# smdesai/mlx-swift-audio

Measured on AMD Instinct MI355X. Metric: audio-sec/s (Whisper large-v3-turbo b=32) at 1/2/4/8 GPU; codec samples/s, higher is better.
Workload: dtype bf16; 1 GPU; Whisper large-v3-turbo bf16, batch=32x30 s synthetic clips per MI355X, log-mel+encode+greedy decode (T=0, timestamps, max_tokens 448, one window per clip), random-init N(0,0.02^2) weights; clips_per_gpu=32, global_batch=32, parallelism=dp1, replicas=3, exchange=none, schedule=pipelined

## Files before the change

mlx-swift-audio_amd/csrc/decode_kernels.hip:

```cpp
#include <cstdlib>

#include <type_traits>
#include "decode.h"

constexpr int ROW_NV = 2;

__device__ __forceinline__ float block256_sum(float v, float* sh) {
  v = wave_sum(v);
  __syncthreads();
  if ((threadIdx.x & 63) == 0) sh[threadIdx.x >> 6] = v;
  __syncthreads();
  return (sh[0] + sh[1]) + (sh[2] + sh[3]);
}

template <typename T>
__device__ __forceinline__ void row_layernorm_store(const f32x4 (&v)[ROW_NV], int nv, int D, const float* __restrict__ gamma,
                                                    const float* __restrict__ beta, uint16_t* __restrict__ h, int row, float* sh) {
  const int tid = threadIdx.x;
  f32x4 gm[ROW_NV], bt[ROW_NV];
#pragma unroll
  for (int i = 0; i < ROW_NV; ++i) {
    const bool in = tid + 256 * i < nv;
    gm[i] = in ? *reinterpret_cast<const f32x4*>(gamma + 4 * (tid + 256 * i)) : (f32x4){0.f, 0.f, 0.f, 0.f};
    bt[i] = in ? *reinterpret_cast<const f32x4*>(beta + 4 * (tid + 256 * i)) : (f32x4){0.f, 0.f, 0.f, 0.f};
// ... 495 lines not shown
  uint32_t wo[NT];
#pragma unroll
  for (int t = 0; t < NT; ++t) wo[t] = wbuf.offset(wp[t]);
  const uint32_t wsb = (uint32_t)ws * 2u;
  int am0 = m0 + r; am0 = am0 < a.M ? am0 : a.M - 1;
  int am1 = m0 + 16 + r; am1 = am1 < a.M ? am1 : a.M - 1;
  const uint16_t* ap0 = a.A + (int64_t)am0 * a.lda + kbeg + 8 * c;
  const uint16_t* ap1 = a.A + (int64_t)am1 * a.lda + kbeg + 8 * c;
  const bool av0 = m0 + r < a.M, av1 = m0 + 16 + r < a.M;
  const s16x8 zfrag = (s16x8){0, 0, 0, 0, 0, 0, 0, 0};
  s16x8 fw[NSTEP][NT], fa0[NSTEP], fa1[NSTEP];
#pragma unroll
  for (int u = 0; u < NSTEP; ++u) {
#pragma unroll
    for (int n = 0; n < NT; ++n) fw[u][n] = wbuf.template load<2>(wo[n] + (uint32_t)u * wsb);
    fa0[u] = zfrag; fa1[u] = zfrag;
    if (av0) fa0[u] = *reinterpret_cast<const s16x8*>(ap0 + 32 * u);
    if (av1) fa1[u] = *reinterpret_cast<const s16x8*>(ap1 + 32 * u);
  }
  __builtin_amdgcn_sched_barrier(0);
  skinny_rstd_prepare(a, rs, m0, wave, lane);
  f32x4 acc[NT][2];
#pragma unroll
  for (int t = 0; t < NT; ++t) { acc[t][0] = (f32x4){0.f, 0.f, 0.f, 0.f}; acc[t][1] = (f32x4){0.f, 0.f, 0.f, 0.f}; }
#pragma unroll
  for (int u = 0; u < NSTEP; ++u)
#pragma unroll
    for (int n = 0; n < NT; ++n) {
      acc[n][0] = T::mfma16(fw[u][n], fa0[u], acc[n][0]);
      acc[n][1] = T::mfma16(fw[u][n], fa1[u], acc[n][1]);
    }
  if (!skinny_wave_reduce<NT, NW>(acc, wave, lane)) return;
  skinny_store<T, MODE, NT>(a, acc, n0, m0, split, lane, rs);
}

template <typename T>
__global__ __launch_bounds__(256) void dec_lnfold(const uint16_t* __restrict__ w, int N, int K, const float* __restrict__ gamma,
                                                  const float* __restrict__ beta, float* __restrict__ c1, float* __restrict__ c2,
                                                  const float* __restrict__ bias) {
  const int lane = threadIdx.x & 63, row = blockIdx.x * 4 + (threadIdx.x >> 6);
  if (row >= N) return;
  const uint16_t* wr = w + (int64_t)row * K;
  float s1 = 0.f, s2 = 0.f;
  for (int k = lane; k < K; k += 64) { const float v = T::to_f32(wr[k]); s1 = fmaf(v, gamma[k], s1); s2 = fmaf(v, beta[k], s2); }
  s1 = wave_sum(s1); s2 = wave_sum(s2);
  if (lane == 0) { c1[row] = s1; c2[row] = s2 + (bias ? bias[row] : 0.f); }
}

int dec_launch_lnfold(const void* w16, int N, int K, const float* gamma, const float* beta, float* c1, float* c2, int dtype, hipStream_t s, const float* bias) {
  if (!w16 || !gamma || !beta || !c1 || !c2 || N <= 0 || K <= 0) return -1;
  if (dtype == MIA_F16) hipLaunchKernelGGL(dec_lnfold<F16>, dim3((N + 3) / 4), dim3(256), 0, s, (const uint16_t*)w16, N, K, gamma, beta, c1, c2, bias);
  else hipLaunchKernelGGL(dec_lnfold<BF16>, dim3((N + 3) / 4), dim3(256), 0, s, (const uint16_t*)w16, N, K, gamma, beta, c1, c2, bias);
  return hipGetLastError() == hipSuccess ? 0 : -1;
}

template <typename T>
__global__ __launch_bounds__(256) void repack_wfrag(const uint16_t* __restrict__ src, uint16_t* __restrict__ dst, int N, int K) {
  const int64_t chunk = (int64_t)blockIdx.x * 256 + threadIdx.x;
  const int ksteps = K >> 5;
  const int64_t total = (int64_t)((N + 15) >> 4) * ksteps * 64;
  if (chunk >= total) return;
  const int lane = (int)(chunk & 63);
  const int64_t tk = chunk >> 6;
  const int kstep = (int)(tk % ksteps), tile = (int)(tk / ksteps);
  const int n = tile * 16 + (lane & 15), k = kstep * 32 + 8 * (lane >> 4);
  s16x8 v = (s16x8){0, 0, 0, 0, 0, 0, 0, 0};
  if (n < N) v = *reinterpret_cast<const s16x8*>(src + (int64_t)n * K + k);
  *reinterpret_cast<s16x8*>(dst + chunk * 8) = v;
}

int dec_launch_repack_wfrag(const void* src, void* dst, int N, int K, hipStream_t s) {
  if (N <= 0 || K <= 0 || K % 32 != 0) return -1;
  const int64_t total = (int64_t)((N + 15) / 16) * (K / 32) * 64;
  hipLaunchKernelGGL(repack_wfrag<BF16>, dim3((unsigned)((total + 255) / 256)), dim3(256), 0, s, (const uint16_t*)src, (uint16_t*)dst, N, K);
  return hipGetLastError() == hipSuccess ? 0 : -1;
}

template <int NW>
struct LnStat {
  static constexpr int RPS = NW >= 8 ? 1 : 8 / NW;
  static constexpr int MAXU = 8;
  f32x2 v[MAXU][RPS];
  int j0, rows;
  bool on;
  __device__ __forceinline__ void issue(const SkinnyArgs& a, int m0, int wave, int lane) {
    on = a.ss_in != nullptr && a.c1 != nullptr;
    const int rg = lane >> 4, l16 = lane & 15;
    j0 = (wave * 4 + rg) * RPS;
    rows = a.M - m0 < 32 ? a.M - m0 : 32;
#pragma unroll
    for (int u = 0; u < MAXU; ++u)
#pragma unroll
      for (int i = 0; i < RPS; ++i) v[u][i] = (f32x2){0.f, 0.f};
    if (!on) return;
    const f32x2* ss = reinterpret_cast<const f32x2*>(a.ss_in);
#pragma unroll
    for (int u = 0; u < MAXU; ++u) {
      const int t = l16 + 16 * u;
      if (t < a.ss_tiles) {
        if (RPS >= 2 && (a.M & 1) == 0) {
#pragma unroll
          for (int i = 0; i + 1 < RPS; i += 2)
            if (j0 + i < rows) {
              const f32x4 p = *reinterpret_cast<const f32x4*>(ss + (int64_t)t * a.M + m0 + j0 + i);
              v[u][i] = (f32x2){p[0], p[1]}; v[u][i + 1] = (f32x2){p[2], p[3]};
            }
        } else {
#pragma unroll
          for (int i = 0; i < RPS; ++i)
            if (j0 + i < rows) v[u][i] = ss[(int64_t)t * a.M + m0 + j0 + i];
        }
      }
    }
  }
  __device__ __forceinline__ void finish(const SkinnyArgs& a, float* st, int lane) {
    if (!on) return;
    const int l16 = lane & 15;
#pragma unroll
    for (int i = 0; i < RPS; ++i) {
      float v1 = 0.f, v2 = 0.f;
#pragma unroll
      for (int u = 0; u < MAXU; ++u) { v1 += v[u][i][0]; v2 += v[u][i][1]; }
      v1 += dpp_f32<0xB1>(v1); v1 += dpp_f32<0x4E>(v1); v1 += dpp_f32<0x141>(v1); v1 += dpp_f32<0x140>(v1);
      v2 += dpp_f32<0xB1>(v2); v2 += dpp_f32<0x4E>(v2); v2 += dpp_f32<0x141>(v2); v2 += dpp_f32<0x140>(v2);
      const int j = j0 + i;
      if (l16 == 0 && j < rows) {
        const float mean = v1 / (float)a.ss_dim;
        const float var = fmaxf(v2 / (float)a.ss_dim - mean * mean, 0.f);
        st[2 * j] = mean; st[2 * j + 1] = rsqrtf(var + a.eps);
      }
    }
  }
};

template <typename T, int NT>
__device__ __forceinline__ void skinny_resid_frag(const SkinnyArgs& a, const f32x4 (&acc)[NT][2], int n0, int m0, int lane) {
  const int r = lane & 15, c = lane >> 4;
#pragma unroll
  for (int t = 0; t < NT; ++t) {
    const int n = n0 + 16 * t + 4 * c;
    const f32x4 gv = *reinterpret_cast<const f32x4*>(a.nw + n);
    f32x4 bv = (f32x4){0.f, 0.f, 0.f, 0.f};
    if (a.bias) bv = *reinterpret_cast<const f32x4*>(a.bias + n);
#pragma unroll
    for (int mt = 0; mt < 2; ++mt) {
      const int m = m0 + mt * 16 + r;
      float s1 = 0.f, s2 = 0.f;
      if (m < a.M) {
        float* xp = a.xres + (int64_t)m * a.N + n;
        f32x4 x = *reinterpret_cast<const f32x4*>(xp);
#pragma unroll
        for (int j = 0; j < 4; ++j) { x[j] += acc[t][mt][j] + bv[j]; s1 += x[j]; s2 += x[j] * x[j]; }
        *reinterpret_cast<f32x4*>(xp) = x;
        *reinterpret_cast<u32x2*>(reinterpret_cast<uint16_t*>(a.out) + afrag_index(m, n, a.N)) =
            (u32x2){pack2<T>(x[0] * gv[0], x[1] * gv[1]), pack2<T>(x[2] * gv[2], x[3] * gv[3])};
      }
      const float a1 = __shfl(s1, r + 16, 64), a2 = __shfl(s1, r + 32, 64), a3 = __shfl(s1, r + 48, 64);
      const float b1 = __shfl(s2, r + 16, 64), b2 = __shfl(s2, r + 32, 64), b3 = __shfl(s2, r + 48, 64);
      if (c == 0 && m < a.M)
        *reinterpret_cast<f32x2*>(a.ss_out + ((int64_t)((n0 >> 4) + t) * a.M + m) * 2) = (f32x2){((s1 + a1) + a2) + a3, ((s2 + b1) + b2) + b3};
    }
  }
}

template <typename T, int MODE, int NT, int NSTEP, int NW>
__global__ __launch_bounds__(64 * NW) void dec_skinny_fflat(SkinnyArgs a) {
  __shared__ float st[64];
  const int lane = threadIdx.x & 63, wave = threadIdx.x >> 6;
  const int split = blockIdx.y, z = blockIdx.z;
  LnStat<NW> lnstat;
  lnstat.issue(a, z * 32, wave, lane);
  const int ksteps = a.K >> 5, tiles = (a.N + 15) >> 4;
  const int ks0 = (split * NW + wave) * NSTEP;
  const uint16_t* wp[NT];
#pragma unroll
  for (int t = 0; t < NT; ++t) {
    int tile = blockIdx.x * NT + t; tile = tile < tiles ? tile : tiles - 1;
    wp[t] = a.W + (((int64_t)tile * ksteps + ks0) * 64 + lane) * 8;
  }
  const uint16_t* ap = a.A + ((((int64_t)z * ksteps + ks0) * 2) * 64 + lane) * 8;
  const SkinnyPre<NT> pre = skinny_prefetch<MODE, NT>(a, blockIdx.x * (16 * NT), z * 32, lane);
  s16x8 fw[NSTEP][NT], fa0[NSTEP], fa1[NSTEP];
  const WFragBuf wb(a);
  const WFragBuf ab(a, 0);
  const uint32_t ao = ab.offset(ap);
  uint32_t wo[NT];
#pragma unroll
  for (int t = 0; t < NT; ++t) wo[t] = wb.offset(wp[t]);
  auto load_all = [&](auto keep_tag) {
    constexpr int AUX = decltype(keep_tag)::value ? 0 : 2;
#pragma unroll
    for (int u = 0; u < NSTEP; ++u) {
#pragma unroll
      for (int n = 0; n < NT; ++n) fw[u][n] = wb.template load<AUX>(wo[n] + 1024u * u);
      fa0[u] = ab.template load<0>(ao + 2048u * u);
      fa1[u] = ab.template load<0>(ao + 2048u * u + 1024u);
    }
  };
  if (a.w_keep) load_all(std::true_type{}); else load_all(std::false_type{});
  __builtin_amdgcn_sched_barrier(0);
  lnstat.finish(a, st, lane);
  f32x4 acc[NT][2];
#pragma unroll
  for (int t = 0; t < NT; ++t) { acc[t][0] = (f32x4){0.f, 0.f, 0.f, 0.f}; acc[t][1] = (f32x4){0.f, 0.f, 0.f, 0.f}; }
#pragma unroll
  for (int u = 0; u < NSTEP; ++u)
#pragma unroll
    for (int n = 0; n < NT; ++n) {
      acc[n][0] = T::mfma16(fw[u][n], fa0[u], acc[n][0]);
      acc[n][1] = T::mfma16(fw[u][n], fa1[u], acc[n][1]);
    }
  if (!skinny_wave_reduce<NT, NW>(acc, wave, lane)) return;
  if constexpr (MODE == SK_RESID) skinny_resid_frag<T, NT>(a, acc, blockIdx.x * (16 * NT), z * 32, lane);
  else skinny_epilogue_v<T, MODE, NT>(a, acc, pre, blockIdx.x * (16 * NT), z * 32, split, lane, st);
}

template <typename T, int MODE, int NT, int KB, int NW>
__global__ __launch_bounds__(64 * NW) void dec_skinny_fring(SkinnyArgs a) {
  __shared__ float st[64];
  const int lane = threadIdx.x & 63, wave = threadIdx.x >> 6;
  const int split = blockIdx.y, z = blockIdx.z;
  LnStat<NW> lnstat;
  lnstat.issue(a, z * 32, wave, lane);
  const int ksteps = a.K >> 5, tiles = (a.N + 15) >> 4;
  const int per_wave = ksteps / (a.S * NW);
  const int ks0 = (split * NW + wave) * per_wave;
  const uint16_t* wp[NT];
#pragma unroll
  for (int t = 0; t < NT; ++t) {
    int tile = blockIdx.x * NT + t; tile = tile < tiles ? tile : tiles - 1;
    wp[t] = a.W + (((int64_t)tile * ksteps + ks0) * 64 + lane) * 8;
  }
  const uint16_t* ap = a.A + ((((int64_t)z * ksteps + ks0) * 2) * 64 + lane) * 8;
  const SkinnyPre<NT> pre = skinny_prefetch<MODE, NT>(a, blockIdx.x * (16 * NT), z * 32, lane);
  f32x4 acc[NT][2];
#pragma unroll
  for (int t = 0; t < NT; ++t) { acc[t][0] = (f32x4){0.f, 0.f, 0.f, 0.f}; acc[t][1] = (f32x4){0.f, 0.f, 0.f, 0.f}; }
  struct Batch { s16x8 w[KB][NT], a0[KB], a1[KB]; };
  const bool keep = a.w_keep != 0;
  const WFragBuf wb(a);
  const WFragBuf ab(a, 0);
  const uint32_t ao = ab.offset(ap);
  uint32_t wo[NT];
#pragma unroll
  for (int t = 0; t < NT; ++t) wo[t] = wb.offset(wp[t]);
  auto load_batch = [&](Batch& t, int ks) {
    auto go = [&](auto keep_tag) {
      constexpr int AUX = decltype(keep_tag)::value ? 0 : 2;
#pragma unroll
      for (int u = 0; u < KB; ++u) {
#pragma unroll
        for (int n = 0; n < NT; ++n) t.w[u][n] = wb.template load<AUX>(wo[n] + 1024u * (uint32_t)(ks + u));
        t.a0[u] = ab.template load<0>(ao + 2048u * (uint32_t)(ks + u));
        t.a1[u] = ab.template load<0>(ao + 2048u * (uint32_t)(ks + u) + 1024u);
      }
    };
    if (keep) go(std::true_type{}); else go(std::false_type{});
  };
  auto mma_batch = [&](const Batch& t) {
#pragma unroll
    for (int u = 0; u < KB; ++u)
#pragma unroll
      for (int n = 0; n < NT; ++n) {
        acc[n][0] = T::mfma16(t.w[u][n], t.a0[u], acc[n][0]);
        acc[n][1] = T::mfma16(t.w[u][n], t.a1[u], acc[n][1]);
      }
  };
  const int nb = per_wave / KB;
  int ks = 0;
  if (nb > 0) {
    Batch b0, b1, b2, b3;
    load_batch(b0, 0);
    if (nb > 1) load_batch(b1, KB);
    if (nb > 2) load_batch(b2, 2 * KB);
    lnstat.finish(a, st, lane);
    for (int i = 0; i < nb; i += 4) {
      if (i + 3 < nb) load_batch(b3, (i + 3) * KB);
      mma_batch(b0);
      if (i + 1 >= nb) break;
      if (i + 4 < nb) load_batch(b0, (i + 4) * KB);
      mma_batch(b1);
      if (i + 2 >= nb) break;
      if (i + 5 < nb) load_batch(b1, (i + 5) * KB);
      mma_batch(b2);
      if (i + 3 >= nb) break;
      if (i + 6 < nb) load_batch(b2, (i + 6) * KB);
      mma_batch(b3);
    }
    ks = nb * KB;
  } else lnstat.finish(a, st, lane);
  for (; ks < per_wave; ++ks) {
    const s16x8 fa0 = *reinterpret_cast<const s16x8*>(ap + 1024 * ks);
    const s16x8 fa1 = *reinterpret_cast<const s16x8*>(ap + 1024 * ks + 512);
#pragma unroll
    for (int n = 0; n < NT; ++n) {
      const s16x8 fw = *reinterpret_cast<const s16x8*>(wp[n] + 512 * ks);
      acc[n][0] = T::mfma16(fw, fa0, acc[n][0]);
      acc[n][1] = T::mfma16(fw, fa1, acc[n][1]);
    }
  }
  if (!skinny_wave_reduce<NT, NW>(acc, wave, lane)) return;
  if constexpr (MODE == SK_RESID) skinny_resid_frag<T, NT>(a, acc, blockIdx.x * (16 * NT), z * 32, lane);
  else skinny_epilogue_v<T, MODE, NT>(a, acc, pre, blockIdx.x * (16 * NT), z * 32, split, lane, st);
}

struct QFrag { const uint32_t* wfrag; const float* stfrag; };

template <typename T> struct QMagic;
template <> struct QMagic<BF16> { static constexpr uint32_t pair = 0x43004300u; static constexpr uint32_t one = 0x3f803f80u; };
template <> struct QMagic<F16> { static constexpr uint32_t pair = 0x64006400u; static constexpr uint32_t one = 0x3c003c00u; };

template <typename T, int MODE, int NT>
__device__ __forceinline__ void skinny_store_tr(const SkinnyArgs& a, const f32x4 (&acc)[NT][2], int n0, int m0, int split, int lane, const float* rs) {
  const int r = lane & 15, c = lane >> 4;
  const bool scaled = a.ss_in != nullptr;
#pragma unroll
  for (int t = 0; t < NT; ++t) {
    const int n = n0 + 16 * t + r;
    const bool nv = n < a.N;
    const float bs = (MODE != SK_PARTIAL && a.bias && nv) ? a.bias[n] : 0.f;
    const float wn = (MODE == SK_RESID && nv) ? a.nw[n] : 0.f;
#pragma unroll
    for (int mt = 0; mt < 2; ++mt) {
#pragma unroll
      for (int i = 0; i < 4; ++i) {
        const int mr = 16 * mt + 4 * c + i, m = m0 + mr;
        const bool mv = m < a.M;
        const float raw = scaled ? acc[t][mt][i] * (mv ? rs[mr] : 0.f) : acc[t][mt][i];
        float v = raw + bs;
        if (MODE == SK_SWIGLU) {
          const float u = dpp_f32<0xB1>(v);
          if (nv && mv && !(r & 1)) reinterpret_cast<uint16_t*>(a.out)[(int64_t)m * a.ldo + (n >> 1)] = T::from_f32((v / (1.0f + __expf(-v))) * u);
          continue;
        }
        if (MODE == SK_RESID) {
          float x = 0.f;
          if (nv && mv) {
            float* xp = a.xres + (int64_t)m * a.N + n;
            x = *xp + v;
            *xp = x;
            reinterpret_cast<uint16_t*>(a.out)[(int64_t)m * a.ldo + n] = T::from_f32(x * wn);
          }
          float q = x * x;
          q += dpp_f32<0xB1>(q); q += dpp_f32<0x4E>(q); q += dpp_f32<0x141>(q); q += dpp_f32<0x140>(q);
          if (r == 0 && mv) a.ss_out[(int64_t)((n0 >> 4) + t) * a.M + m] = q;
          continue;
        }
        if (!nv || !mv) continue;
        if (MODE == SK_PARTIAL) reinterpret_cast<float*>(a.out)[((int64_t)split * a.M + m) * a.N + n] = raw;
        else if (MODE == SK_OUTF32) reinterpret_cast<float*>(a.out)[(int64_t)m * a.ldo + n] = v;
        else reinterpret_cast<uint16_t*>(a.out)[(int64_t)m * a.ldo + n] = T::from_f32(v);
      }
    }
  }
}

template <typename T, int MODE, int NT, int NW, bool M16, int NP>
__global__ __launch_bounds__(64 * NW) void skinny_gemm_qi(SkinnyArgs a, QFrag q) {
  __shared__ float rs[32];
  const int lane = threadIdx.x & 63;
  const int wave = __builtin_amdgcn_readfirstlane(threadIdx.x >> 6);
  const int tile0 = blockIdx.x * NT;
  const int n0 = tile0 * 16;
  const int split = blockIdx.y;
  const int m0 = blockIdx.z * 32;
  const int nblk = a.K >> 7;
  const int bc = nblk / (a.S * NW);
  const int b0 = (split * NW + wave) * bc;
  const int n_tiles = (a.N + 15) >> 4;
  const int r = lane & 15, c = lane >> 4;
  const bool av0 = m0 + r < a.M, av1 = !M16 && m0 + 16 + r < a.M;
  const uint16_t* ap0 = a.A + (int64_t)(av0 ? m0 + r : 0) * a.lda + 8 * c;
  const uint16_t* ap1 = a.A + (int64_t)(av1 ? m0 + 16 + r : 0) * a.lda + 8 * c;
  const u32x4* wp[NT];
  const f32x4* sp[NT];
#pragma unroll
  for (int t = 0; t < NT; ++t) {
    const int tl = tile0 + t < n_tiles ? tile0 + t : n_tiles - 1;
    wp[t] = reinterpret_cast<const u32x4*>(q.wfrag) + ((int64_t)tl * nblk) * (NP * 64) + lane;
    sp[t] = reinterpret_cast<const f32x4*>(q.stfrag) + ((int64_t)tl * nblk) * 16 + r;
  }
  const __amdgpu_buffer_rsrc_t rw = __builtin_amdgcn_make_buffer_rsrc(const_cast<uint32_t*>(q.wfrag), (short)0, (int)((unsigned)n_tiles * (unsigned)nblk * (NP * 64 * 16u)), 0x00020000);
  const __amdgpu_buffer_rsrc_t rst = __builtin_amdgcn_make_buffer_rsrc(const_cast<float*>(q.stfrag), (short)0, (int)((unsigned)n_tiles * (unsigned)nblk * 256u), 0x00020000);
  uint32_t wo[NT], so[NT];
#pragma unroll
  for (int t = 0; t < NT; ++t) {
    wo[t] = (uint32_t)((const char*)wp[t] - (const char*)q.wfrag);
    so[t] = (uint32_t)((const char*)sp[t] - (const char*)q.stfrag);
  }
  f32x4 acc[NT][2];
#pragma unroll
  for (int t = 0; t < NT; ++t) { acc[t][0] = (f32x4){0.f, 0.f, 0.f, 0.f}; acc[t][1] = (f32x4){0.f, 0.f, 0.f, 0.f}; }
  const s16x8 zfrag = (s16x8){0, 0, 0, 0, 0, 0, 0, 0};
  struct Blk { u32x4 w[NT][NP]; f32x4 st[NT]; s16x8 a0[4], a1[4]; };
  auto load_blk = [&](Blk& b, int blk) {
#pragma unroll
    for (int t = 0; t < NT; ++t) {
#pragma unroll
      for (int p = 0; p < NP; ++p) b.w[t][p] = __builtin_bit_cast(u32x4, __builtin_amdgcn_raw_buffer_load_b128(rw, (int)(wo[t] + (uint32_t)(blk * NP + p) * 1024u), 0, 2));
      b.st[t] = __builtin_bit_cast(f32x4, __builtin_amdgcn_raw_buffer_load_b128(rst, (int)(so[t] + (uint32_t)blk * 256u), 0, 2));
    }
#pragma unroll
    for (int st = 0; st < 4; ++st) {
      b.a0[st] = zfrag;
      if (av0) b.a0[st] = *reinterpret_cast<const s16x8*>(ap0 + (int64_t)blk * 128 + 32 * st);
      if (!M16) { b.a1[st] = zfrag; if (av1) b.a1[st] = *reinterpret_cast<const s16x8*>(ap1 + (int64_t)blk * 128 + 32 * st); }
    }
  };
  const f32x4 zero4 = (f32x4){0.f, 0.f, 0.f, 0.f};
  const s16x8 ones = __builtin_bit_cast(s16x8, (u32x4){QMagic<T>::one, QMagic<T>::one, QMagic<T>::one, QMagic<T>::one});
  auto unpack = [](uint32_t word) -> s16x8 {
    return __builtin_bit_cast(s16x8, (u32x4){(word & 0x000f000fu) | QMagic<T>::pair, ((word >> 4) & 0x000f000fu) | QMagic<T>::pair,
                                             ((word >> 8) & 0x000f000fu) | QMagic<T>::pair, ((word >> 12) & 0x000f000fu) | QMagic<T>::pair});
  };
  auto mma_blk = [&](const Blk& b) {
#pragma unroll
    for (int g = 0; g < 2; ++g) {
      f32x4 A0 = T::mfma16(b.a0[2 * g], ones, zero4), A1 = zero4;
      A0 = T::mfma16(b.a0[2 * g + 1], ones, A0);
      if (!M16) { A1 = T::mfma16(b.a1[2 * g], ones, zero4); A1 = T::mfma16(b.a1[2 * g + 1], ones, A1); }
#pragma unroll
      for (int t = 0; t < NT; ++t) {
        f32x4 P0[NP], P1[NP];
#pragma unroll
        for (int p = 0; p < NP; ++p) {
          const s16x8 f0 = unpack(b.w[t][p][2 * g]), f1 = unpack(b.w[t][p][2 * g + 1]);
          P0[p] = T::mfma16(b.a0[2 * g], f0, zero4);
          P0[p] = T::mfma16(b.a0[2 * g + 1], f1, P0[p]);
          if (!M16) { P1[p] = T::mfma16(b.a1[2 * g], f0, zero4); P1[p] = T::mfma16(b.a1[2 * g + 1], f1, P1[p]); }
        }
        const float sc = b.st[t][2 * g], tt = b.st[t][2 * g + 1];
#pragma unroll
        for (int i = 0; i < 4; ++i) {
          const float p0 = NP == 2 ? __builtin_fmaf(16.0f, P0[NP - 1][i], P0[0][i]) : P0[0][i];
          acc[t][0][i] = __builtin_fmaf(sc, p0, __builtin_fmaf(tt, A0[i], acc[t][0][i]));
          if (!M16) {
            const float p1 = NP == 2 ? __builtin_fmaf(16.0f, P1[NP - 1][i], P1[0][i]) : P1[0][i];
            acc[t][1][i] = __builtin_fmaf(sc, p1, __builtin_fmaf(tt, A1[i], acc[t][1][i]));
          }
        }
      }
    }
  };
  Blk k0, k1, k2;
  if (bc > 0) load_blk(k0, b0);
  if (bc > 1) load_blk(k1, b0 + 1);
  skinny_rstd_prepare(a, rs, m0, wave, lane);
  for (int i = 0; i < bc; i += 3) {
    if (i + 2 < bc) load_blk(k2, b0 + i + 2);
    mma_blk(k0);
    if (i + 1 >= bc) break;
    if (i + 3 < bc) load_blk(k0, b0 + i + 3);
    mma_blk(k1);
    if (i + 2 >= bc) break;
    if (i + 4 < bc) load_blk(k1, b0 + i + 4);
    mma_blk(k2);
  }
  if (!skinny_wave_reduce<NT, NW>(acc, wave, lane)) return;
  skinny_store_tr<T, MODE, NT>(a, acc, n0, m0, split, lane, rs);
}

constexpr int DEC_MAX_KEYS = 1536;

template <typename T, int U, bool NTL>
__global__ __launch_bounds__(256) void dec_attention(const uint16_t* __restrict__ q, const uint16_t* __restrict__ kc,
                                                     const uint16_t* __restrict__ vc, uint16_t* __restrict__ out,
                                                     const int32_t* __restrict__ pos_arr, int fixed_keys, int cap_keys, int H,
                                                     float scale, float* __restrict__ qk_out, const int32_t* __restrict__ head_slot,
                                                     int n_slots, int qk_ctx) {
  __shared__ float sc[DEC_MAX_KEYS];
  __shared__ float red[4][64];
  __shared__ float red2[8];
  const int tid = threadIdx.x, lane = tid & 63, wave = tid >> 6;
  const int h = blockIdx.x, b = blockIdx.y;
  const int D = H * 64;
  const int nk = fixed_keys > 0 ? fixed_keys : pos_arr[b] + 1;
  const int c = lane & 7, g = lane >> 3;
  const uint16_t* kb = kc + ((int64_t)b * H + h) * cap_keys * 64;
  const uint16_t* vb = vc + ((int64_t)b * H + h) * cap_keys * 64;
  float qf[8];
  {
    const s16x8 qv = *reinterpret_cast<const s16x8*>(q + (int64_t)b * D + h * 64 + c * 8);
#pragma unroll
    for (int j = 0; j < 8; ++j) qf[j] = T::to_f32((uint16_t)qv[j]);
  }
  const __amdgpu_buffer_rsrc_t rk = __builtin_amdgcn_make_buffer_rsrc(const_cast<uint16_t*>(kb), (short)0, cap_keys * 128, 0x00020000);
  const __amdgpu_buffer_rsrc_t rv = __builtin_amdgcn_make_buffer_rsrc(const_cast<uint16_t*>(vb), (short)0, cap_keys * 128, 0x00020000);
  auto load_trip = [&](s16x8 (&dst)[U], const __amdgpu_buffer_rsrc_t& base, int k0) {
#pragma unroll
    for (int u = 0; u < U; ++u) {
      int key = k0 + 8 * u + g; key = key < nk ? key : nk - 1;
      dst[u] = __builtin_bit_cast(s16x8, __builtin_amdgcn_raw_buffer_load_b128(base, key * 128 + c * 16, 0, NTL ? 2 : 0));
    }
  };
  constexpr int TRIP = 32 * U;
  {
    int k0 = wave * (8 * U);
    s16x8 kv[U], kn[U];
    if (k0 < nk) load_trip(kv, rk, k0);
    for (; k0 < nk; k0 += TRIP) {
      const bool more = k0 + TRIP < nk;
      if (more) load_trip(kn, rk, k0 + TRIP);
#pragma unroll
      for (int u = 0; u < U; ++u) {
        float dot = 0.f;
#pragma unroll
        for (int j = 0; j < 8; ++j) dot += qf[j] * T::to_f32((uint16_t)kv[u][j]);
        dot += dpp_xor1(dot);
        dot += dpp_xor2(dot);
        dot += dpp_half_mirror(dot);
        const int key = k0 + 8 * u + g;
        if (c == 0 && key < nk) sc[key] = dot * scale;
      }
      if (more) {
#pragma unroll
        for (int u = 0; u < U; ++u) kv[u] = kn[u];
      }
    }
  }
  s16x8 vv[U], vn[U];
  if (wave * (8 * U) < nk) load_trip(vv, rv, wave * (8 * U));
  __syncthreads();
  if (qk_out && head_slot[h] >= 0) {
    float* dst = qk_out + (((int64_t)b * n_slots + head_slot[h]) * qk_ctx + pos_arr[b]) * nk;
    for (int i = tid; i < nk; i += 256) dst[i] = sc[i];
  }
  float m = -INFINITY;
  for (int i = tid; i < nk; i += 256) m = fmaxf(m, sc[i]);
  m = wave_max(m);
  if (lane == 0) red2[wave] = m;
  __syncthreads();
  m = fmaxf(fmaxf(red2[0], red2[1]), fmaxf(red2[2], red2[3]));
  float sum = 0.f;
  for (int i = tid; i < nk; i += 256) { const float p = __expf(sc[i] - m); sc[i] = p; sum += p; }
  sum = wave_sum(sum);
  if (lane == 0) red2[4 + wave] = sum;
  __syncthreads();
  sum = (red2[4] + red2[5]) + (red2[6] + red2[7]);
  float acc[8];
#pragma unroll
  for (int j = 0; j < 8; ++j) acc[j] = 0.f;
  for (int k0 = wave * (8 * U); k0 < nk; k0 += TRIP) {
    const bool more = k0 + TRIP < nk;
    if (more) load_trip(vn, rv, k0 + TRIP);
    float pw[U];
#pragma unroll
    for (int u = 0; u < U; ++u) {
      const int key = k0 + 8 * u + g;
      pw[u] = key < nk ? sc[key] : 0.f;
    }
#pragma unroll
    for (int u = 0; u < U; ++u)
#pragma unroll
      for (int j = 0; j < 8; ++j) acc[j] += pw[u] * T::to_f32((uint16_t)vv[u][j]);
    if (more) {
#pragma unroll
      for (int u = 0; u < U; ++u) vv[u] = vn[u];
    }
  }
#pragma unroll
  for (int j = 0; j < 8; ++j) {
    acc[j] += dpp_xor8(acc[j]);
    acc[j] += __shfl_xor(acc[j], 16, 64);
    acc[j] += __shfl_xor(acc[j], 32, 64);
  }
  if (g == 0) {
#pragma unroll
    for (int j = 0; j < 8; ++j) red[wave][c * 8 + j] = acc[j];
  }
  __syncthreads();
  if (tid < 64) {
    const float o = ((red[0][tid] + red[1][tid]) + (red[2][tid] + red[3][tid])) / sum;
    out[afrag_index(b, h * 64 + tid, D)] = T::from_f32(o);
  }
}

struct HeadBufs {
  const float* logits;
  int32_t* tokens;
  int32_t* n_gen;
  int32_t* finished;
  int32_t* last_ts;
  float* sum_logprob;
  int32_t* n_logprob;
  float* no_speech;
  const uint32_t* suppress;
  const float* uniforms;
  DecClip clip;
};

constexpr int HEAD_NPT = 52;
struct ArgMax { float v; int i; };
__device__ __forceinline__ ArgMax amax(ArgMax a, ArgMax b) {
  return (b.v > a.v || (b.v == a.v && b.i < a.i)) ? b : a;
}
__device__ __forceinline__ ArgMax wave_amax(ArgMax a) {
#define AMAX_STEP(CTRL) { const ArgMax b{dpp_f32<CTRL>(a.v), dpp_i32<CTRL>(a.i)}; a = amax(a, b); }
  AMAX_STEP(0xB1) AMAX_STEP(0x4E) AMAX_STEP(0x141) AMAX_STEP(0x140)
#undef AMAX_STEP
  ArgMax r = ArgMax{lane_f32(a.v, 0), __builtin_amdgcn_readlane(a.i, 0)};
  r = amax(r, ArgMax{lane_f32(a.v, 16), __builtin_amdgcn_readlane(a.i, 16)});
  r = amax(r, ArgMax{lane_f32(a.v, 32), __builtin_amdgcn_readlane(a.i, 32)});
  r = amax(r, ArgMax{lane_f32(a.v, 48), __builtin_amdgcn_readlane(a.i, 48)});
  return r;
}

// ... 224 lines not shown
#pragma unroll
  for (int u = 0; u < HEAD_NPT2; ++u) { const int i = base + tid + 256 * u; x[u] = i < V ? lg[i] : -INFINITY; }
  const HeadRule r = head_rule(hb, p, b);
  if (!r.active) return;
  const int nw = (V + 31) / 32;
  const uint32_t* bits = hb.suppress + (r.num_gen == 0 ? nw : 0);
  auto maskedA = [&](int i) -> bool {
    if ((bits[i >> 5] >> (i & 31)) & 1u) return true;
    if (p.timestamps) {
      if (i == p.no_timestamps) return true;
      if (r.sup_ts_all && i >= tsb) return true;
      if (r.sup_text_below_eot && i < p.eot) return true;
      if (i >= tsb && i < r.ts_floor) return true;
      if (r.sup_below_tsb && i < tsb) return true;
      if (i > r.max_first) return true;
    }
    return false;
  };
  float mx_text = -INFINITY, mx_ts = -INFINITY;
  ArgMax bA{-INFINITY, 0x7fffffff}, bB{-INFINITY, 0x7fffffff};
  unsigned okA = 0u;
#pragma unroll
  for (int u = 0; u < HEAD_NPT2; ++u) {
    const int i = base + tid + 256 * u;
    if (i >= V) continue;
    if (i >= tsb) mx_ts = fmaxf(mx_ts, x[u]); else mx_text = fmaxf(mx_text, x[u]);
    if (r.decide && !maskedA(i)) {
      okA |= 1u << u;
      bA = amax(bA, ArgMax{x[u], i});
      if (i >= tsb) bB = amax(bB, ArgMax{x[u], i});
    }
  }
  mx_text = wave_max(mx_text); mx_ts = wave_max(mx_ts);
  bA = wave_amax(bA); bB = wave_amax(bB);
  if (lane == 0) { shf[wave][0] = mx_text; shf[wave][1] = mx_ts; sha[wave][0] = bA.v; shai[wave][0] = bA.i; sha[wave][1] = bB.v; shai[wave][1] = bB.i; }
  __syncthreads();
  mx_text = shf[0][0]; mx_ts = shf[0][1]; bA = ArgMax{sha[0][0], shai[0][0]}; bB = ArgMax{sha[0][1], shai[0][1]};
  for (int w2 = 1; w2 < 4; ++w2) {
    mx_text = fmaxf(mx_text, shf[w2][0]); mx_ts = fmaxf(mx_ts, shf[w2][1]);
    bA = amax(bA, ArgMax{sha[w2][0], shai[w2][0]}); bB = amax(bB, ArgMax{sha[w2][1], shai[w2][1]});
  }
  const float mx_all = fmaxf(mx_text, mx_ts);
  __syncthreads();
  float s_all = 0.f, s_ts = 0.f, fA = 0.f, fB = 0.f;
#pragma unroll
  for (int u = 0; u < HEAD_NPT2; ++u) {
    const int i = base + tid + 256 * u;
    if (i >= V) continue;
    s_all += __expf(x[u] - mx_all);
    if (r.heuristic && i >= tsb) s_ts += __expf(x[u] - mx_ts);
    if ((okA >> u) & 1u) {
      fA += __expf(x[u] - bA.v);
      if (r.heuristic && i >= tsb) fB += __expf(x[u] - bB.v);
    }
  }
  s_all = wave_sum(s_all); s_ts = wave_sum(s_ts); fA = wave_sum(fA); fB = wave_sum(fB);
  if (lane == 0) { shf[wave][0] = s_all; shf[wave][1] = s_ts; shf[wave][2] = fA; shf[wave][3] = fB; }
  __syncthreads();
  if (tid == 0) {
    s_all = s_ts = fA = fB = 0.f;
    for (int w2 = 0; w2 < 4; ++w2) { s_all += shf[w2][0]; s_ts += shf[w2][1]; fA += shf[w2][2]; fB += shf[w2][3]; }
    parts[b * HEAD_SPLIT + k] = HeadPart{mx_text, mx_ts, s_all, s_ts, bA.v, bB.v, fA, fB, bA.i, bB.i};
  }
}

struct NextEmbed { const uint16_t* emb; const float* pos_emb; const float* gamma; const float* beta; float* x; uint16_t* h; int D; };

template <typename T>
__global__ __launch_bounds__(256) void dec_head_final(HeadBufs hb, DecodeParams p, const HeadPart* __restrict__ parts, NextEmbed ne) {
  __shared__ int s_newpos;
  __shared__ float sh[4];
  const int b = blockIdx.x, tid = threadIdx.x;
  float mx_text = -INFINITY, mx_ts = -INFINITY, s_all = 0.f, s_ts = 0.f, fA = 0.f, fB = 0.f;
  ArgMax bA{-INFINITY, 0x7fffffff}, bB{-INFINITY, 0x7fffffff};
  const HeadRule r = head_rule(hb, p, b);
  if (tid < 64 && r.active) {
    HeadPart me{-INFINITY, -INFINITY, 0.f, 0.f, -INFINITY, -INFINITY, 0.f, 0.f, 0x7fffffff, 0x7fffffff};
    if (tid < HEAD_SPLIT) me = parts[b * HEAD_SPLIT + tid];
    mx_text = wave_max(me.mx_text); mx_ts = wave_max(me.mx_ts);
    bA = wave_amax(ArgMax{me.bAv, me.bAi}); bB = wave_amax(ArgMax{me.bBv, me.bBi});
    const float mx_all = fmaxf(mx_text, mx_ts);
    const float ml = fmaxf(me.mx_text, me.mx_ts);
    s_all = wave_sum(ml > -INFINITY ? me.s_all * __expf(ml - mx_all) : 0.f);
    s_ts = wave_sum(me.mx_ts > -INFINITY ? me.s_ts * __expf(me.mx_ts - mx_ts) : 0.f);
    fA = wave_sum(me.bAv > -INFINITY ? me.fA * __expf(me.bAv - bA.v) : 0.f);
    fB = wave_sum(me.bBv > -INFINITY ? me.fB * __expf(me.bBv - bB.v) : 0.f);
  }
  if (tid == 0) {
    int newpos = -1;
    const int pos = hb.clip.pos[b];
    const int n_initial = hb.clip.n_init[b], sot_index = hb.clip.sot_idx[b];
    if (!r.active) {
      if (r.cur_len < n_initial) newpos = pos + 1;
    } else {
      const int V = p.V, tsb = p.timestamp_begin;
      const float* lg = hb.logits + (int64_t)b * V;
      int32_t* toks = hb.tokens + (int64_t)b * p.n_ctx;
      const float mx_all = fmaxf(mx_text, mx_ts);
      const float lse = mx_all + __logf(s_all);
      if (pos == sot_index) hb.no_speech[b] = __expf(lg[p.no_speech] - lse);
      if (!r.decide) newpos = pos + 1;
      else {
        bool useB = false;
        if (r.heuristic) {
          const float ts_lse = (mx_ts - lse) + __logf(s_ts);
          const float max_text = mx_text - lse;
          useB = ts_lse > max_text;
        }
        const ArgMax best = useB ? bB : bA;
        const float fsum = useB ? fB : fA;
        const bool all_masked = best.i == 0x7fffffff;
        const int next = all_masked ? 0 : best.i;
        if (next != p.eot) {
          hb.sum_logprob[b] += all_masked ? __int_as_float(0x7fc00000) : (lg[next] - best.v) - __logf(fsum);
          hb.n_logprob[b] += 1;
        }
        toks[r.cur_len] = next;
        hb.n_gen[b] = r.num_gen + 1;
        if (next > tsb) hb.last_ts[b] = next;
        int cap = p.max_tokens - n_initial;
        if (p.max_new_tokens > 0 && p.max_new_tokens < cap) cap = p.max_new_tokens;
        if (next == p.eot || r.num_gen + 1 >= cap) hb.finished[b] = 1;
        else newpos = pos + 1;
      }
    }
    if (newpos >= 0) hb.clip.pos[b] = newpos;
    s_newpos = newpos;
  }
  __syncthreads();
  const int np_ = s_newpos;
  if (np_ < 0 || np_ >= p.n_ctx) return;
  const int D = ne.D, nv = D >> 2;
  const int tok = hb.tokens[(int64_t)b * p.n_ctx + np_];
  const uint16_t* e = ne.emb + (int64_t)tok * D;
  const float* pe = ne.pos_emb + (int64_t)np_ * D;
  float* xr = ne.x + (int64_t)b * D;
  f32x4 v[ROW_NV];
#pragma unroll
  for (int i = 0; i < ROW_NV; ++i) {
    const int c = tid + 256 * i;
    if (c < nv) {
      const s16x4 ev = *reinterpret_cast<const s16x4*>(e + 4 * c);
      const f32x4 pv = *reinterpret_cast<const f32x4*>(pe + 4 * c);
#pragma unroll
      for (int j = 0; j < 4; ++j) v[i][j] = T::to_f32((uint16_t)ev[j]) + pv[j];
      *reinterpret_cast<f32x4*>(xr + 4 * c) = v[i];
    } else v[i] = (f32x4){0.f, 0.f, 0.f, 0.f};
  }
  row_layernorm_store<T>(v, nv, D, ne.gamma, ne.beta, ne.h, b, sh);
}

__global__ void dec_finalize(const int32_t* __restrict__ tokens, const int32_t* __restrict__ n_gen,
                             const float* __restrict__ sum_lp, const int32_t* __restrict__ n_lp, int32_t* __restrict__ out_tokens,
                             int32_t* __restrict__ out_n, float* __restrict__ out_avg, const int32_t* __restrict__ n_init, DecodeParams p) {
  const int b = blockIdx.x;
  const int32_t* t = tokens + (int64_t)b * p.n_ctx + n_init[b];
  __shared__ int n_keep;
  if (threadIdx.x == 0) {
    int n = n_gen[b];
    for (int i = 0; i < n; ++i) if (t[i] == p.eot) { n = i; break; }
    n_keep = n;
    out_n[b] = n;
    out_avg[b] = n_lp[b] > 0 ? sum_lp[b] / (float)n_lp[b] : 0.0f;
  }
  __syncthreads();
  for (int i = threadIdx.x; i < p.max_tokens; i += blockDim.x) out_tokens[(int64_t)b * p.max_tokens + i] = i < n_keep ? t[i] : 0;
}

int dec_launch_embed_ln(mia_whisper* w, const LNW& ln, hipStream_t s) {
  const int D = w->dims.n_text_state;
  if (w->dtype == MIA_F16)
    hipLaunchKernelGGL(dec_embed_ln<F16>, dim3(w->cur_B), dim3(256), 0, s, w->tokens, (const uint16_t*)w->tok_emb, w->dec_pos, ln.g, ln.b, w->dx, (uint16_t*)w->dh, w->clip.pos, D, w->dims.n_text_ctx);
  else
    hipLaunchKernelGGL(dec_embed_ln<BF16>, dim3(w->cur_B), dim3(256), 0, s, w->tokens, (const uint16_t*)w->tok_emb, w->dec_pos, ln.g, ln.b, w->dx, (uint16_t*)w->dh, w->clip.pos, D, w->dims.n_text_ctx);
  return 0;
}

int dec_launch_reduce_ln(mia_whisper* w, int S, const float* bias, const LNW& ln, hipStream_t s) {
  const int D = w->dims.n_text_state;
  if (w->dtype == MIA_F16)
    hipLaunchKernelGGL(dec_reduce_ln<F16>, dim3(w->cur_B), dim3(256), 0, s, w->partial, S, w->cur_B, bias, ln.g, ln.b, w->dx, (uint16_t*)w->dh, D);
  else
    hipLaunchKernelGGL(dec_reduce_ln<BF16>, dim3(w->cur_B), dim3(256), 0, s, w->partial, S, w->cur_B, bias, ln.g, ln.b, w->dx, (uint16_t*)w->dh, D);
  return 0;
}

template <typename T, int MODE>
static bool skinny_flat_try(const SkinnyArgs& a, hipStream_t s) {
  const int tiles = (a.N + 15) / 16, zb = (a.M + 31) / 32;
  const int64_t wgs = (int64_t)tiles * a.S * zb;
  if (a.K % (128 * a.S) != 0 || wgs > 1024 || a.K / a.S < 512) return false;
  const int per_split = a.K / a.S;
  const dim3 grid(tiles, a.S, zb);
#define FLAT(NSTEP_)                                                                                                  \
  if (per_split == 4 * 32 * NSTEP_) {                                                                                 \
    hipLaunchKernelGGL((dec_skinny_flat<T, MODE, 1, NSTEP_, 4>), grid, dim3(256), 0, s, a);                            \
    return true;                                                                                                      \
  }
  FLAT(10) FLAT(5) FLAT(8) FLAT(6) FLAT(4)
#undef FLAT
  return false;
}

template <typename T>
static void skinny_launch_t(const SkinnyArgs& a, int mode, hipStream_t s) {
  switch (mode) {
    case SK_OUTF32: break;
    case SK_OUT16: if (skinny_flat_try<T, SK_OUT16>(a, s)) return; break;
    case SK_PARTIAL: if (skinny_flat_try<T, SK_PARTIAL>(a, s)) return; break;
    case SK_SWIGLU: if (skinny_flat_try<T, SK_SWIGLU>(a, s)) return; break;
    case SK_RESID: break;
    default: if (skinny_flat_try<T, SK_QKV>(a, s)) return; break;
  }
  if (mode == SK_OUTF32) {
    dim3 grid((a.N + 63) / 64, a.S, (a.M + 31) / 32);
    hipLaunchKernelGGL((dec_skinny_gemm<T, SK_OUTF32, 4, 2, 1>), grid, dim3(64), 0, s, a);
    return;
  }
  dim3 grid((a.N + 15) / 16, a.S, (a.M + 31) / 32);
  const bool wide = (int64_t)grid.x * grid.y * grid.z <= 1024 && a.K % (128 * a.S) == 0 && a.K / a.S >= 512;
#define SK_LAUNCH(MODE_)                                                                                              \
  do {                                                                                                                \
    if (wide) hipLaunchKernelGGL((dec_skinny_gemm<T, MODE_, 1, 2, 4>), grid, dim3(256), 0, s, a);                      \
    else hipLaunchKernelGGL((dec_skinny_gemm<T, MODE_, 1, 4, 1>), grid, dim3(64), 0, s, a);                            \
  } while (0)
  switch (mode) {
    case SK_OUT16: SK_LAUNCH(SK_OUT16); break;
    case SK_PARTIAL: SK_LAUNCH(SK_PARTIAL); break;
    case SK_SWIGLU: SK_LAUNCH(SK_SWIGLU); break;
    case SK_RESID:
      if (a.K % 1024 == 0 && a.K >= 8192) hipLaunchKernelGGL((dec_skinny_gemm<T, SK_RESID, 1, 2, 16>), grid, dim3(1024), 0, s, a);
      else if (a.K % 256 == 0 && a.K >= 2048) hipLaunchKernelGGL((dec_skinny_gemm<T, SK_RESID, 1, 2, 8>), grid, dim3(512), 0, s, a);
      else SK_LAUNCH(SK_RESID);
      break;
    default: SK_LAUNCH(SK_QKV); break;
  }
#undef SK_LAUNCH
}

int skinny_gemm_launch(const SkinnyArgs& a, int mode, int dtype, hipStream_t s) {
  if (a.K % (32 * a.S) != 0 || a.lda % 8 != 0) return -1;
  if (mode == SK_SWIGLU && (a.N & 3)) return -1;
  if (mode == SK_RESID && (a.S != 1 || (a.N & 15) || (a.ldo & 3) || !a.xres || !a.nw || !a.ss_out)) return -1;
  if (a.ss_in && (a.ss_tiles <= 0 || a.ss_dim <= 0)) return -1;
  if (dtype == MIA_F16) skinny_launch_t<F16>(a, mode, s); else skinny_launch_t<BF16>(a, mode, s);
  return 0;
}


template <typename T, bool M16, int NP>
static void skinny_qi_launch_m(const SkinnyArgs& a, const QFrag& q, int mode, hipStream_t s) {
  const int tiles = (a.N + 15) / 16, nblk = a.K / 128;
  const int zb = (a.M + 31) / 32;
  const int per_split = nblk / a.S;
  const bool nt4 = (int64_t)tiles * a.S * zb >= 16384 || (a.M > 16 && (int64_t)((tiles + 3) / 4) * a.S * zb >= 192);
  int nw = 1;
  for (int cand : {4, 3, 2}) if (per_split % cand == 0 && (per_split / cand >= 2 || cand == 2)) { nw = cand; break; }
  const bool head41 = mode == SK_OUTF32 && tiles >= 4096 && a.M <= 16;
#define QI_GO(MODE_, NT_, NW_) hipLaunchKernelGGL((skinny_gemm_qi<T, MODE_, NT_, NW_, M16, NP>), dim3((tiles + NT_ - 1) / NT_, a.S, zb), dim3(64 * NW_), 0, s, a, q)
#define QI_LAUNCH(MODE_)                                                                                   \
  do {                                                                                                     \
    if (head41) QI_GO(MODE_, 4, 1);                                                                        \
    else if (nt4) { if (per_split % 4 == 0) QI_GO(MODE_, 4, 4); else QI_GO(MODE_, 4, 1); }                  \
    else if (nw == 4) QI_GO(MODE_, 1, 4); else if (nw == 3) QI_GO(MODE_, 1, 3);                             \
    else if (nw == 2) QI_GO(MODE_, 1, 2); else QI_GO(MODE_, 1, 1);                                          \
  } while (0)
  switch (mode) {
    case SK_OUTF32: QI_LAUNCH(SK_OUTF32); break;
    case SK_OUT16: QI_LAUNCH(SK_OUT16); break;
    case SK_SWIGLU: QI_LAUNCH(SK_SWIGLU); break;
    case SK_RESID:
      if (!nt4 && per_split % 16 == 0 && per_split >= 64) QI_GO(SK_RESID, 1, 16);
      else if (!nt4 && per_split % 8 == 0) QI_GO(SK_RESID, 1, 8);
      else QI_LAUNCH(SK_RESID);
      break;
    default: QI_LAUNCH(SK_PARTIAL); break;
  }
#undef QI_LAUNCH
#undef QI_GO
}

template <typename T>
static void skinny_qi_launch_t(const SkinnyArgs& a, const QFrag& q, int bits, int mode, hipStream_t s) {
  if (bits == 8) { if (a.M <= 16) skinny_qi_launch_m<T, true, 2>(a, q, mode, s); else skinny_qi_launch_m<T, false, 2>(a, q, mode, s); }
  else { if (a.M <= 16) skinny_qi_launch_m<T, true, 1>(a, q, mode, s); else skinny_qi_launch_m<T, false, 1>(a, q, mode, s); }
}

int skinny_gemm_q_launch(const SkinnyArgs& a, const uint32_t* wfrag, const float* stfrag, int bits, int mode, int dtype, hipStream_t s) {
  if (a.K % (128 * a.S) != 0 || a.lda % 8 != 0 || !wfrag || !stfrag) return -1;
  if (bits != 4 && bits != 8) return -1;
  if (mode != SK_OUT16 && mode != SK_OUTF32 && mode != SK_PARTIAL && mode != SK_SWIGLU && mode != SK_RESID) return -1;
  if (mode == SK_SWIGLU && (a.N & 3)) return -1;
  if (mode == SK_RESID && (a.S != 1 || (a.N & 15) || !a.xres || !a.nw || !a.ss_out)) return -1;
  if (a.ss_in && (a.ss_tiles <= 0 || a.ss_dim <= 0)) return -1;
  const QFrag q{wfrag, stfrag};
  if (dtype == MIA_F16) skinny_qi_launch_t<F16>(a, q, bits, mode, s); else skinny_qi_launch_t<BF16>(a, q, bits, mode, s);
  return hipGetLastError() == hipSuccess ? 0 : -1;
}

template <typename T, int MODE>
static int skinny_frag_launch_m(const SkinnyArgs& a, hipStream_t s) {
  const int tiles = (a.N + 15) / 16, zb = (a.M + 31) / 32, ksteps = a.K / 32;
  if constexpr (MODE == SK_OUTF32) {
    hipLaunchKernelGGL((dec_skinny_fring<T, MODE, 4, 2, 1>), dim3((tiles + 3) / 4, a.S, zb), dim3(64), 0, s, a);
    return 0;
  } else {
    const int per_split = ksteps / a.S;
    const dim3 grid(tiles, a.S, zb);
    if constexpr (MODE == SK_RESID) {
      if (per_split == 160) { hipLaunchKernelGGL((dec_skinny_fring<T, MODE, 1, 2, 16>), grid, dim3(1024), 0, s, a); return 0; }
      if (per_split == 80) { hipLaunchKernelGGL((dec_skinny_fflat<T, MODE, 1, 10, 8>), grid, dim3(512), 0, s, a); return 0; }
      if (per_split == 40) { hipLaunchKernelGGL((dec_skinny_fflat<T, MODE, 1, 5, 8>), grid, dim3(512), 0, s, a); return 0; }
      if (per_split % 16 == 0 && per_split >= 64) { hipLaunchKernelGGL((dec_skinny_fring<T, MODE, 1, 1, 16>), grid, dim3(1024), 0, s, a); return 0; }
      if (per_split % 8 == 0 && per_split >= 16) { hipLaunchKernelGGL((dec_skinny_fring<T, MODE, 1, 1, 8>), grid, dim3(512), 0, s, a); return 0; }
    }
    const int NW = per_split % 4 == 0 ? 4 : per_split % 2 == 0 ? 2 : 1;
    const int nstep = per_split / NW;
#define FF(NS_)                                                                                                       \
    if (NW == 4 && nstep == NS_) { hipLaunchKernelGGL((dec_skinny_fflat<T, MODE, 1, NS_, 4>), grid, dim3(256), 0, s, a); return 0; }
    FF(10) FF(5) FF(8) FF(6) FF(4) FF(3) FF(2) FF(1)
#undef FF
    if (NW == 4) hipLaunchKernelGGL((dec_skinny_fring<T, MODE, 1, 1, 4>), grid, dim3(256), 0, s, a);
    else if (NW == 2) hipLaunchKernelGGL((dec_skinny_fring<T, MODE, 1, 1, 2>), grid, dim3(128), 0, s, a);
    else hipLaunchKernelGGL((dec_skinny_fring<T, MODE, 1, 1, 1>), grid, dim3(64), 0, s, a);
    return 0;
  }
}

template <typename T>
static int skinny_frag_launch_t(const SkinnyArgs& a, int mode, hipStream_t s) {
  switch (mode) {
    case SK_OUT16: return skinny_frag_launch_m<T, SK_OUT16>(a, s);
    case SK_OUTF32: return skinny_frag_launch_m<T, SK_OUTF32>(a, s);
    case SK_PARTIAL: return skinny_frag_launch_m<T, SK_PARTIAL>(a, s);
    case SK_QKV: return skinny_frag_launch_m<T, SK_QKV>(a, s);
    case SK_RESID: return skinny_frag_launch_m<T, SK_RESID>(a, s);
    default: return -1;
  }
}

int dec_launch_skinny(mia_whisper* w, const SkinnyArgs& a, int mode, hipStream_t s) {
  if (!a.A || !a.W || !a.out || a.M <= 0 || a.N <= 0 || a.S <= 0 || a.K % (32 * a.S) != 0) return -1;
  if (mode == SK_QKV && (a.D % 64 != 0 || a.N != 3 * a.D || (a.ldo & 3) || !a.cache_k || !a.cache_v || !a.pos)) return -1;
  if (mode == SK_OUT16 && a.out_frag && a.N % 32 != 0) return -1;
  if (mode == SK_RESID && (a.S != 1 || a.N % 32 != 0 || !a.xres || !a.nw || !a.ss_out)) return -1;
  if (a.c1 && (!a.c2 || !a.ss_in || a.ss_tiles <= 0 || a.ss_dim <= 0)) return -1;
  return w->dtype == MIA_F16 ? skinny_frag_launch_t<F16>(a, mode, s) : skinny_frag_launch_t<BF16>(a, mode, s);
}

int dec_launch_attention(mia_whisper* w, const void* q, const void* kc, const void* vc, void* out, int fixed_keys, int cap_keys,
                         hipStream_t s, float* qk_out, const int32_t* head_slot, int n_slots, int qk_ctx) {
  if (cap_keys > DEC_MAX_KEYS) return -1;
  dim3 grid(w->dims.n_text_head, w->cur_B), block(256);
#define ATT(T_, U_, NTL_)                                                                                                            \
  hipLaunchKernelGGL((dec_attention<T_, U_, NTL_>), grid, block, 0, s, (const uint16_t*)q, (const uint16_t*)kc, (const uint16_t*)vc,   \
                     (uint16_t*)out, w->clip.pos, fixed_keys, cap_keys, w->dims.n_text_head, 0.125f, qk_out, head_slot, n_slots, qk_ctx)
  if (w->dtype == MIA_F16) { if (fixed_keys > 0) ATT(F16, 4, true); else ATT(F16, 4, false); }
  else { if (fixed_keys > 0) ATT(BF16, 4, true); else ATT(BF16, 4, false); }
#undef ATT
  return 0;
}

bool dec_head_is_split(const DecodeParams& p) {
  return p.greedy && !p.head_single && p.V <= 256 * HEAD_NPT2 * HEAD_SPLIT;
}

__global__ __launch_bounds__(256) void dec_trace_logits(const float* __restrict__ logits, const int32_t* __restrict__ pos, const int32_t* __restrict__ clips,
                                                        float* __restrict__ trace, int V, int n_ctx) {
  const int slot = blockIdx.y, b = clips[slot];
  const int p = pos[b];
  if (p < 0 || p >= n_ctx) return;
  const float* src = logits + (int64_t)b * V;
  float* dst = trace + ((int64_t)slot * n_ctx + p) * V;
  for (int i = blockIdx.x * 256 + threadIdx.x; i < V; i += gridDim.x * 256) dst[i] = src[i];
}

int dec_launch_trace(mia_whisper* w, hipStream_t s) {
  if (!w->trace || w->trace_n <= 0) return -1;
  hipLaunchKernelGGL(dec_trace_logits, dim3(32, w->trace_n), dim3(256), 0, s, w->logits, w->clip.pos, w->trace_clips, w->trace, w->dims.n_vocab, w->dims.n_text_ctx);
  return 0;
}

int dec_launch_head(mia_whisper* w, int32_t* last_ts, const DecodeParams& p, hipStream_t s) {
  if (p.V > 1024 * HEAD_NPT) return -1;
  HeadBufs hb{w->logits, w->tokens, w->n_gen, w->finished, last_ts, w->sum_logprob, w->n_logprob, w->no_speech, w->suppress_bits, w->uniforms, w->clip};
  if (dec_head_is_split(p)) {
    HeadPart* parts = reinterpret_cast<HeadPart*>(w->partial);
    hipLaunchKernelGGL(dec_head_partial, dim3(HEAD_SPLIT, w->cur_B), dim3(256), 0, s, hb, p, parts);
    const LNW& ln0 = w->dec[0].attn_ln;
    NextEmbed ne{(const uint16_t*)w->tok_emb, w->dec_pos, ln0.g, ln0.b, w->dx, (uint16_t*)w->dh, w->dims.n_text_state};
    if (w->dtype == MIA_F16) hipLaunchKernelGGL(dec_head_final<F16>, dim3(w->cur_B), dim3(256), 0, s, hb, p, (const HeadPart*)parts, ne);
    else hipLaunchKernelGGL(dec_head_final<BF16>, dim3(w->cur_B), dim3(256), 0, s, hb, p, (const HeadPart*)parts, ne);
    return 0;
  }
  hipLaunchKernelGGL(dec_head, dim3(w->cur_B), dim3(1024), 0, s, hb, p);
  return 0;
}

int dec_launch_finalize(mia_whisper* w, int32_t* out_n, const DecodeParams& p, hipStream_t s) {
  hipLaunchKernelGGL(dec_finalize, dim3(w->cur_B), dim3(256), 0, s, w->tokens, w->n_gen, w->sum_logprob, w->n_logprob, w->out_tokens, out_n, w->out_avg, w->clip.n_init, p);
  return 0;
}
```

Baseline: 4696 audio-sec/s.

## Add dedicated vocab-projection GEMM kernel with buffer-load ring pipelining

Adds a new dec_vocab_gemm kernel for the fp32-output skinny GEMM (the vocab logits projection) when there is no K split and no c1 term. It uses buffer-resource loads with cache-policy hints for the weight stream and a four-deep register ring of batched fragment loads to overlap memory with MFMA. It also allows each wave to cover several N tiles, either strided or contiguous. The aim is to stream the large vocab weight matrix closer to bandwidth. The cost is higher register pressure, and each tile runs its own epilogue.

```diff
diff --git a/mlx-swift-audio_amd/csrc/decode_kernels.hip b/mlx-swift-audio_amd/csrc/decode_kernels.hip
--- a/mlx-swift-audio_amd/csrc/decode_kernels.hip
+++ b/mlx-swift-audio_amd/csrc/decode_kernels.hip
@@ -821,6 +821,91 @@
   if (!skinny_wave_reduce<NT, NW>(acc, wave, lane)) return;
   if constexpr (MODE == SK_RESID) skinny_resid_frag<T, NT>(a, acc, blockIdx.x * (16 * NT), z * 32, lane);
   else skinny_epilogue_v<T, MODE, NT>(a, acc, pre, blockIdx.x * (16 * NT), z * 32, split, lane, st);
+}
+
+template <typename T, int NT, int KB, int WPG, bool STRIDED>
+__global__ __launch_bounds__(64 * WPG) void dec_vocab_gemm(SkinnyArgs a) {
+  const int lane = threadIdx.x & 63;
+  const int g = blockIdx.x * WPG + (threadIdx.x >> 6), G = gridDim.x * WPG;
+  const int z = blockIdx.z;
+  const int ksteps = a.K >> 5, tiles = (a.N + 15) >> 4;
+  int tl[NT];
+#pragma unroll
+  for (int t = 0; t < NT; ++t) tl[t] = STRIDED ? g + t * G : g * NT + t;
+  const WFragBuf wb(a);
+  const WFragBuf ab(a, 0);
+  const uint32_t ao = ab.offset(a.A + (((int64_t)z * ksteps * 2) * 64 + lane) * 8);
+  uint32_t wo[NT];
+#pragma unroll
+  for (int t = 0; t < NT; ++t) {
+    const int tile = tl[t] < tiles ? tl[t] : tiles - 1;
+    wo[t] = wb.offset(a.W + (((int64_t)tile * ksteps) * 64 + lane) * 8);
+  }
+  f32x4 acc[NT][2];
+#pragma unroll
+  for (int t = 0; t < NT; ++t) { acc[t][0] = (f32x4){0.f, 0.f, 0.f, 0.f}; acc[t][1] = (f32x4){0.f, 0.f, 0.f, 0.f}; }
+  struct Batch { s16x8 w[KB][NT], a0[KB], a1[KB]; };
+  const bool keep = a.w_keep != 0;
+  auto load_batch = [&](Batch& t, int ks) {
+    auto go = [&](auto keep_tag) {
+      constexpr int AUX = decltype(keep_tag)::value ? 0 : 2;
+#pragma unroll
+      for (int u = 0; u < KB; ++u) {
+#pragma unroll
+        for (int n = 0; n < NT; ++n) t.w[u][n] = wb.template load<AUX>(wo[n] + 1024u * (uint32_t)(ks + u));
+        t.a0[u] = ab.template load<0>(ao + 2048u * (uint32_t)(ks + u));
+        t.a1[u] = ab.template load<0>(ao + 2048u * (uint32_t)(ks + u) + 1024u);
+      }
+    };
+    if (keep) go(std::true_type{}); else go(std::false_type{});
+  };
+  auto mma_batch = [&](const Batch& t) {
+#pragma unroll
+    for (int u = 0; u < KB; ++u)
+#pragma unroll
+      for (int n = 0; n < NT; ++n) {
+        acc[n][0] = T::mfma16(t.w[u][n], t.a0[u], acc[n][0]);
+        acc[n][1] = T::mfma16(t.w[u][n], t.a1[u], acc[n][1]);
+      }
+  };
+  const int nb = ksteps / KB;
+  int ks = 0;
+  if (nb > 0) {
+    Batch b0, b1, b2, b3;
+    load_batch(b0, 0);
+    if (nb > 1) load_batch(b1, KB);
+    if (nb > 2) load_batch(b2, 2 * KB);
+    for (int i = 0; i < nb; i += 4) {
+      if (i + 3 < nb) load_batch(b3, (i + 3) * KB);
+      mma_batch(b0);
+      if (i + 1 >= nb) break;
+      if (i + 4 < nb) load_batch(b0, (i + 4) * KB);
+      mma_batch(b1);
+      if (i + 2 >= nb) break;
+      if (i + 5 < nb) load_batch(b1, (i + 5) * KB);
+      mma_batch(b2);
+      if (i + 3 >= nb) break;
+      if (i + 6 < nb) load_batch(b2, (i + 6) * KB);
+      mma_batch(b3);
+    }
+    ks = nb * KB;
+  }
+  for (; ks < ksteps; ++ks) {
+    const s16x8 fa0 = ab.template load<0>(ao + 2048u * (uint32_t)ks);
+    const s16x8 fa1 = ab.template load<0>(ao + 2048u * (uint32_t)ks + 1024u);
+#pragma unroll
+    for (int n = 0; n < NT; ++n) {
+      const s16x8 fw = wb.template load<0>(wo[n] + 1024u * (uint32_t)ks);
+      acc[n][0] = T::mfma16(fw, fa0, acc[n][0]);
+      acc[n][1] = T::mfma16(fw, fa1, acc[n][1]);
+    }
+  }
+#pragma unroll
+  for (int t = 0; t < NT; ++t) {
+    const f32x4 one[1][2] = {{acc[t][0], acc[t][1]}};
+    const SkinnyPre<1> pre = skinny_prefetch<SK_OUTF32, 1>(a, tl[t] * 16, z * 32, lane);
+    skinny_epilogue_v<T, SK_OUTF32, 1>(a, one, pre, tl[t] * 16, z * 32, 0, lane);
+  }
 }
 
 struct QFrag { const uint32_t* wfrag; const float* stfrag; };
@@ -1651,6 +1736,10 @@
 static int skinny_frag_launch_m(const SkinnyArgs& a, hipStream_t s) {
   const int tiles = (a.N + 15) / 16, zb = (a.M + 31) / 32, ksteps = a.K / 32;
   if constexpr (MODE == SK_OUTF32) {
+    if (a.S == 1 && !a.c1) {
+      hipLaunchKernelGGL((dec_vocab_gemm<T, 4, 4, 1, false>), dim3((tiles + 3) / 4, 1, zb), dim3(64), 0, s, a);
+      return 0;
+    }
     hipLaunchKernelGGL((dec_skinny_fring<T, MODE, 4, 2, 1>), dim3((tiles + 3) / 4, a.S, zb), dim3(64), 0, s, a);
     return 0;
   } else {
```

New measurement: 4700 audio-sec/s, median of 6. No clear change (+0.1%).
